# nayuki/DEFLATE-library-Java

Measured on AMD Instinct MI355X. Metric: input MiB/s (compress+decompress), higher is better.
Workload: dtype u8

## Files before the change

### deflate-library-java_amd/csrc/hip/inflate_wave.hpp

```cpp
#pragma once

namespace wv {
using namespace inf;

enum : uint32_t { K_LIT = 0, K_LEN = 1, K_EOB = 2, K_BAD = 3 };

struct Shared {
    Tabs t;
    uint8_t lens[320];
    uint16_t cl_tab[128];
    uint32_t exit_[64];
    uint8_t kind_[64];
    uint64_t h_pos, h_d0;
    uint32_t h_err, h_bfinal, h_btype, h_len, h_numlit, h_numdist;
};

struct PhArr {
    uint32_t cp[7][64];
    uint32_t end[7][64];
    uint32_t cnt[7][64];
    uint8_t kr[7][64];
};

__device__ __forceinline__ uint32_t lit_entry(uint32_t sym, uint32_t len) {
// ... 898 lines not shown
                tok_e<false>(lo[k], hi[k], en[k], p[k], t, ed, e, nb, tk);
                if (tk.kind > K_LEN) { l[k] = false; O[k].kr = tk.kind == K_EOB ? (T_EOB << 5) : ((T_ERR << 5) | tk.val); }
                else c[k] += tk.n;
            }
        }
    }
#pragma unroll
    for (int k = 0; k < N; k++) {
        Tok tk;
        if (l[k] && run_to(v, p[k], t, ed, e, nb, c[k], tk)) O[k].kr = tk.kind == K_EOB ? (T_EOB << 5) : ((T_ERR << 5) | tk.val);
        O[k].end = p[k]; O[k].cnt = c[k];
    }
}

__device__ __forceinline__ uint32_t esc_index(uint32_t lo, uint32_t hi, uint32_t esc4) {
    const uint32_t tl = (lo & esc4) ^ esc4, th = (hi & esc4) ^ esc4;
    const uint32_t zl = (tl - 0x01010101u) & ~tl & 0x80808080u, zh = (th - 0x01010101u) & ~th & 0x80808080u;
    return zl ? (uint32_t)__builtin_ctz(zl) >> 3 : zh ? 4u + ((uint32_t)__builtin_ctz(zh) >> 3) : 8u;
}
template <int N>
__device__ __forceinline__ void phase_multi_esc(const Lv& v, const Tabs& t, bool ed, uint32_t nb, uint32_t s0, uint32_t e,
                                                uint32_t esc4, PhOut (&O)[N]) {
    uint32_t p[N], c[N];
    bool l[N];
#pragma unroll
    for (int k = 0; k < N; k++) phase_first(v, t, ed, nb, s0 + k, e, p[k], c[k], O[k], l[k]);
    for (;;) {
        bool f[N], any = false;
#pragma unroll
        for (int k = 0; k < N; k++) { f[k] = l[k] && p[k] < e; any = any || f[k]; }
        if (!any) break;
        uint32_t lo[N], hi[N];
#pragma unroll
        for (int k = 0; k < N; k++) {
            const uint32_t pp = f[k] ? p[k] : p[0];
            const uint32_t* qk = v.p + ((pp >> 5) - v.rw) * 64;
            const uint32_t a = qk[0], wb = qk[64], cw = qk[128];
            lo[k] = __builtin_amdgcn_alignbit(wb, a, pp & 31);
            hi[k] = __builtin_amdgcn_alignbit(cw, wb, pp & 31);
        }
#pragma unroll
        for (int k = 0; k < N; k++) {
            if (!f[k]) continue;
            const uint32_t q = (e - p[k] + 7) >> 3, qi = (nb - min(nb, p[k])) >> 3;
            const uint32_t tt = min(min(esc_index(lo[k], hi[k], esc4), q), qi);
            if (tt) { p[k] += 8 * tt; c[k] += tt; continue; }
            Tok tk;
            tok_e<true>(lo[k], hi[k], t.lit[lo[k] & ((1u << LB) - 1u)], p[k], t, ed, e, nb, tk);
            if (tk.kind > K_LEN) { l[k] = false; O[k].kr = tk.kind == K_EOB ? (T_EOB << 5) : ((T_ERR << 5) | tk.val); }
            else c[k] += tk.n;
        }
    }
#pragma unroll
    for (int k = 0; k < N; k++) { O[k].end = p[k]; O[k].cnt = c[k]; }
}
__device__ __forceinline__ uint32_t flat8_mask(const Tabs& t, int lane) {
    uint64_t L[4];
#pragma unroll
    for (uint32_t i = 0; i < 4; i++) L[i] = __ballot((t.lit[(uint32_t)lane + 64 * i] & 0x800001FFu) == 0x80000088u);
    uint32_t m4 = 0;
#pragma unroll
    for (uint32_t kk = 0; kk < 3; kk++) {
        const uint32_t M = (1u << (8 - kk)) - 1u;
        bool same = true;
#pragma unroll
        for (uint32_t i = 0; i < 4; i++) same = same && __ballot((((uint32_t)lane + 64 * i) & M) != M) == L[i];
        if (same && !m4) m4 = M * 0x01010101u;
    }
    return m4;
}

__device__ __forceinline__ uint32_t sel8(const uint32_t (&v)[8], uint32_t i) {
    uint32_t r = v[0];
#pragma unroll
    for (uint32_t k = 1; k < 8; k++) r = i == k ? v[k] : r;
    return r;
}
__device__ __forceinline__ uint32_t phase_of(uint32_t d, uint32_t fbl, uint32_t fbh) {
    if (d < 8) return d;
    uint32_t r = 8;
#pragma unroll
    for (uint32_t f = 0; f < 8; f++) {
        const uint32_t fo = ((f < 4 ? fbl : fbh) >> (8 * (f & 3))) & 0xFFu;
        if (r == 8 && fo == d) r = f | 16u;
    }
    return r;
}
__device__ __forceinline__ uint32_t map_compose(uint32_t A, uint32_t B) {
    uint32_t r = 0;
#pragma unroll
    for (uint32_t f = 0; f < 8; f++) {
        const uint32_t bf = (B >> (4 * f)) & 15u;
        const uint32_t v = bf < 8 ? (A >> (4 * bf)) & 15u : 8u;
        r |= v << (4 * f);
    }
    return r;
}

__device__ __noinline__ void round_decode_phased(const In& in, const Tabs& t, bool ed, uint64_t rs, uint64_t E,
                                                 Shared& S, Stage& stg, int lane, Seg& out, uint32_t& first_term,
                                                 uint32_t& nfix, Geo& g, uint32_t esc4) {
    g = make_geo(in, rs, E);
    stage_round(in, g, stg, lane);
    const Lv v = make_lv(stg, g, lane);
    const uint32_t nb = g.nb;
    uint32_t s, e;
    lane_seg(g, lane, s, e);
    uint32_t endv[8], cntv[8], fbcv[8], krv[8];
    uint32_t fbl = 0, fbh = 0;
    constexpr uint32_t G = 2;
#pragma unroll 1
    for (uint32_t f = 0; f < 8; f += G) {
        PhOut P[G];
        if (esc4) phase_multi_esc<G>(v, t, ed, nb, s + f, e, esc4, P);
        else phase_multi<G>(v, t, ed, nb, s + f, e, P);
#pragma unroll
        for (uint32_t h = 0; h < G; h++) {
            const uint32_t g = f + h;
#pragma unroll
            for (uint32_t k = 0; k < 8; k++) {
                endv[k] = k == g ? P[h].end : endv[k];
                cntv[k] = k == g ? P[h].cnt : cntv[k];
                fbcv[k] = k == g ? P[h].fbc : fbcv[k];
                krv[k] = k == g ? P[h].kr : krv[k];
            }
            const uint32_t fo = (P[h].fb != NOCP && P[h].fb - s < 255u) ? P[h].fb - s : 255u;
            if (g < 4) fbl |= fo << (8 * g); else fbh |= fo << (8 * (g - 4));
        }
    }
    uint32_t Q = 0;
#pragma unroll
    for (uint32_t f = 0; f < 8; f++) {
        const uint32_t x = __shfl_up(endv[f], 1, 64);
        const uint32_t vv = phase_of(x - s, fbl, fbh) & 15u;
        if (lane > 0) Q |= vv << (4 * f);
    }
#pragma unroll
    for (int k = 1; k < 64; k <<= 1) {
        const uint32_t B = __shfl_up(Q, k, 64);
        if (lane >= k) Q = map_compose(Q, B);
    }
    const uint32_t myph = Q & 15u;
    const uint32_t xsel = myph < 8 ? sel8(endv, myph) : NOCP;
    uint32_t x = __shfl_up(xsel, 1, 64);
    if (lane == 0) x = s;
    SegR r;
    r.start = x; r.end = x; r.cnt = 0; r.kind = T_ERR; r.reason = R_INTERNAL;
    bool known = false;
    if (myph < 8) {
        const uint32_t pc = phase_of(x - s, fbl, fbh);
        const uint32_t f = pc & 15u;
        if (f == myph) {
            known = true;
            const uint32_t kr = sel8(krv, f);
            r.end = sel8(endv, f);
            r.cnt = sel8(cntv, f) - ((pc & 16u) ? sel8(fbcv, f) : 0u);
            r.kind = kr >> 5; r.reason = kr & 31u;
        }
    }
    const uint64_t km = __ballot(!known);
    const uint32_t u = km ? (uint32_t)__builtin_ctzll(km) : 64u;
    const uint64_t tm = __ballot(known && r.kind != T_EXIT);
    const uint32_t t0 = tm ? (uint32_t)__builtin_ctzll(tm) : 64u;
    first_term = min(t0, 64u);
    if (u < t0) {
        S.exit_[lane] = r.end;
        __syncthreads();
        first_term = 64;
        for (uint32_t j = u; j < 64 && first_term == 64; j++) {
            nfix++;
            if ((uint32_t)lane == j) {
                const uint32_t st = j ? (uint32_t)S.exit_[j - 1] : s;
                uint32_t en, cn, kr, fb, fbc;
                if (esc4) {
                    PhOut P1[1];
                    phase_multi_esc<1>(v, t, ed, nb, st, e, esc4, P1);
                    en = P1[0].end; cn = P1[0].cnt; kr = P1[0].kr;
                } else {
                    phase_run(v, t, ed, nb, st, e, en, cn, kr, fb, fbc);
                }
                r.start = st; r.end = en; r.cnt = cn; r.kind = kr >> 5; r.reason = kr & 31u;
                S.exit_[lane] = en;
                S.kind_[lane] = r.kind;
            }
            __syncthreads();
            if (S.kind_[j] != T_EXIT) first_term = j;
        }
    }
    out.start = g.base + r.start; out.end = g.base + r.end; out.cnt = r.cnt;
    out.kind = r.kind; out.reason = r.reason;
}

__device__ __forceinline__ uint64_t wave_sum_u64(uint64_t x) {
#pragma unroll
    for (int o = 32; o > 0; o >>= 1) x += __shfl_xor((unsigned long long)x, o, 64);
    return x;
}
__device__ __forceinline__ uint64_t wave_excl_u64(uint64_t v, int lane) {
    uint64_t x = v;
#pragma unroll
    for (int o = 1; o < 64; o <<= 1) {
        const uint64_t y = __shfl_up((unsigned long long)x, o, 64);
        if (lane >= o) x += y;
    }
    return x - v;
}

__device__ __forceinline__ bool is_cand(const uint64_t* cands, uint32_t ncand, uint64_t b, uint32_t* idx = nullptr) {
    uint32_t lo = 0, hi = ncand;
    while (lo < hi) { const uint32_t mid = (lo + hi) >> 1; if (cands[mid] < b) lo = mid + 1; else hi = mid; }
    if (idx) *idx = lo;
    return lo < ncand && cands[lo] == b;
}

__device__ __forceinline__ uint64_t next_cand(const uint64_t* cands, uint32_t ncand, uint64_t b, uint64_t limit) {
    uint32_t lo = 0, hi = ncand;
    while (lo < hi) { const uint32_t mid = (lo + hi) >> 1; if (cands[mid] <= b) lo = mid + 1; else hi = mid; }
    const uint64_t nx = lo < ncand ? cands[lo] : NONE;
    return min(nx, limit);
}

struct CandCur {
    const uint64_t* c;
    uint32_t n, i;
    uint64_t v;
    __device__ __forceinline__ void init(const uint64_t* cands, uint32_t ncand, uint64_t b) {
        c = cands; n = ncand;
        uint32_t lo = 0, hi = n;
        while (lo < hi) { const uint32_t mid = (lo + hi) >> 1; if (c[mid] < b) lo = mid + 1; else hi = mid; }
        i = lo;
        v = i < n ? c[i] : NONE;
    }
    __device__ __forceinline__ bool at(uint64_t b, uint32_t* idx) {
        while (v < b) { i++; v = i < n ? c[i] : NONE; }
        *idx = i;
        return v == b;
    }
    __device__ __forceinline__ uint64_t after(uint64_t b, uint64_t limit) {
        while (v <= b) { i++; v = i < n ? c[i] : NONE; }
        return min(v, limit);
    }
};

typedef __attribute__((address_space(1))) uint8_t gu8;
typedef __attribute__((address_space(1))) uint32_t gu32;
typedef __attribute__((address_space(1))) uint64_t gu64;

#ifdef NDFL_EMIT_NOSTORE
#define NDFL_OA(x) ((x) & 0xFFFull)
#else
#define NDFL_OA(x) (x)
#endif
typedef uint32_t u32x4v __attribute__((ext_vector_type(4)));
typedef __attribute__((address_space(1))) u32x4v gu128;
struct Wr {
    uint64_t acc;
    uint32_t an;
    uint64_t dst;
    uint32_t q0, q1, q2, hn;
};
__device__ __forceinline__ void wr_init(Wr& w, uint64_t dst) {
    w.acc = 0; w.an = 0; w.dst = dst;
    w.q0 = 0; w.q1 = 0; w.q2 = 0; w.hn = 0;
}
__device__ __forceinline__ void wr_drain(Wr& w, gu8* out) {
    if (w.hn) {
        gu8* d = out + NDFL_OA(w.dst - 4 * w.hn);
        if (w.hn >= 2) *(gu64*)d = (uint64_t)w.q0 | ((uint64_t)w.q1 << 32);
        if (w.hn == 1) *(gu32*)d = w.q0;
        if (w.hn == 3) *(gu32*)(d + 8) = w.q2;
        w.hn = 0;
    }
}
__device__ __forceinline__ void wr_lit(Wr& w, gu8* out, uint32_t val, uint32_t n) {
    w.acc |= (uint64_t)val << (8 * w.an);
    w.an += n;
    if (w.an >= 4) {
        const uint32_t word = (uint32_t)w.acc;
        if (w.hn == 3) {
            *(gu128*)(out + NDFL_OA(w.dst - 12)) = u32x4v{w.q0, w.q1, w.q2, word};
            w.hn = 0;
        } else {
            w.q0 = w.hn == 0 ? word : w.q0;
            w.q1 = w.hn == 1 ? word : w.q1;
            w.q2 = w.hn == 2 ? word : w.q2;
            w.hn++;
        }
        w.acc >>= 32;
        w.an -= 4;
        w.dst += 4;
    }
}
__device__ __forceinline__ void wr_flush_word(Wr& w, gu8* out) {
    wr_drain(w, out);
    if (w.an) {
        *(gu32*)(out + NDFL_OA(w.dst)) = (uint32_t)w.acc;
        w.dst += w.an;
        w.acc = 0;
        w.an = 0;
    }
}
__device__ __forceinline__ void wr_flush_exact(Wr& w, gu8* out) {
    wr_drain(w, out);
    for (uint32_t k = 0; k < w.an; k++) out[NDFL_OA(w.dst + k)] = (uint8_t)(w.acc >> (8 * k));
    w.dst += w.an;
    w.acc = 0;
    w.an = 0;
}
__device__ __forceinline__ uint64_t ld8(const gu8* p) { return *(const gu64*)p; }
__device__ __forceinline__ uint32_t ld4(const gu8* p) { return *(const gu32*)p; }
__device__ __forceinline__ void wr_copy(gu8* out, uint64_t dst, uint32_t len, uint32_t dist, uint32_t& lastb) {
    gu8* d = out + NDFL_OA(dst);
    const gu8* sp = out + NDFL_OA(dst - dist);
    if (dist == 1) {
        const uint32_t v4 = lastb * 0x01010101u;
        if (len >= 16) {
            const u32x4v x = {v4, v4, v4, v4};
            uint32_t k = 0;
            for (; k + 16 <= len; k += 16) *(gu128*)(d + k) = x;
            if (k < len) *(gu128*)(d + len - 16) = x;
            return;
        }
        if (len >= 4) {
            uint32_t k = 0;
            for (; k + 4 <= len; k += 4) *(gu32*)(d + k) = v4;
            if (k < len) *(gu32*)(d + len - 4) = v4;
        } else {
            for (uint32_t k = 0; k < len; k++) d[k] = (uint8_t)lastb;
        }
        return;
    }
    if (dist >= 16 && len >= 16) {
        uint32_t k = 0;
        u32x4v x = {0, 0, 0, 0};
        for (; k + 16 <= len; k += 16) { x = *(const gu128*)(sp + k); *(gu128*)(d + k) = x; }
        if (k < len) { x = *(const gu128*)(sp + len - 16); *(gu128*)(d + len - 16) = x; }
        lastb = x.w >> 24;
        return;
    }
    if (dist >= 8 && len >= 8) {
        uint32_t k = 0;
        uint64_t x = 0;
        for (; k + 8 <= len; k += 8) { x = ld8(sp + k); *(gu64*)(d + k) = x; }
        if (k < len) { x = ld8(sp + len - 8); *(gu64*)(d + len - 8) = x; }
        lastb = (uint32_t)(x >> 56);
        return;
    }
    if (dist >= 4 && len >= 4) {
        uint32_t k = 0, x = 0;
        for (; k + 4 <= len; k += 4) { x = ld4(sp + k); *(gu32*)(d + k) = x; }
        if (k < len) { x = ld4(sp + len - 4); *(gu32*)(d + len - 4) = x; }
        lastb = x >> 24;
        return;
    }
    uint32_t b = lastb;
    for (uint32_t k = 0; k < len; k++) { b = sp[k]; d[k] = (uint8_t)b; }
    lastb = b;
}

}

extern "C" __global__ void __launch_bounds__(64)
ndfl_inflate_hdr_kernel(const uint32_t* w, uint64_t nwords, uint64_t nbits, const uint64_t* cands, uint32_t ncand,
                        wv::HdrRec* rec, uint32_t* flat_list, uint32_t* nflat, uint32_t* flat_flag) {
    using namespace wv;
    __shared__ __attribute__((aligned(16))) uint32_t lens[64][80];
    __shared__ uint16_t clt[64][128];
    __shared__ uint32_t win[8 * 64];
    const uint32_t lane = threadIdx.x;
    const uint32_t k = blockIdx.x * 64 + lane;
    if (k >= ncand) return;
    const In in{w, nwords, nbits};
    for (uint32_t q = 0; q < 80; q++) lens[lane][q] = 0;
    const uint64_t p = cands[k];
    Hdr h;
    parse_hdr_core<RdWin>(in, p, (uint8_t*)lens[lane], clt[lane], h, win + lane);
    HdrRec* r = rec + k;
    for (uint32_t q = 0; q < 80; q += 4)
        *(uint4*)&r->lens[q] = make_uint4(lens[lane][q], lens[lane][q + 1], lens[lane][q + 2], lens[lane][q + 3]);
    r->h = h;
    r->at = p;
    uint32_t c8 = 0;
    bool bad = false;
    for (uint32_t q = 0; q < 72; q++) {
        const uint32_t v = lens[lane][q];
#pragma unroll
        for (uint32_t b = 0; b < 4; b++) {
            const uint32_t l = (v >> (8 * b)) & 0xFFu;
            c8 += l == 8 ? 1u : 0u;
            bad = bad || (l - 1u < 7u) || (l == 8 && q >= 64);
        }
    }
    const uint32_t esc = 256u - min(c8, 256u);
    const uint32_t kk = esc == 1 ? 1u : esc == 2 ? 2u : esc == 4 ? 3u : 0u;
    r->flat = (flat_list && h.err == 0 && h.btype == 2 && !bad) ? kk : 0u;
    r->pad = 0;
    if (flat_flag) flat_flag[k] = r->flat;
    if (flat_list) {
        const uint64_t m = __ballot(r->flat != 0);
        uint32_t b = 0;
        if (lane == 0 && m) b = atomicAdd(nflat, (uint32_t)__popcll(m));
        b = __shfl(b, 0, 64);
        if (r->flat) flat_list[b + (uint32_t)__popcll(m & ((1ull << lane) - 1ull))] = k;
    }
}

#ifndef NDFL_COUNT_WPE
#define NDFL_COUNT_WPE 3
#endif
namespace wv {
#ifndef NDFL_FLAT_OTHER_MAX
#define NDFL_FLAT_OTHER_MAX 64
#endif
#ifndef NDFL_FLAT_K
#define NDFL_FLAT_K 4
#endif
#ifndef NDFL_FLAT_PRIO
#define NDFL_FLAT_PRIO 1
#endif
#ifdef NDFL_FLAT_PROF
__device__ unsigned long long g_flat_prof[4];
#endif
constexpr uint32_t FLAT_ESC_WORD = 64;
static_assert(FLAT_ESC_WORD + 64 * 64 / 4 <= SW * 64, "flat escape tables in the stage");

__device__ __forceinline__ uint32_t flat_esc_entry(const TabsG& t, uint32_t kk, uint32_t x) {
    const uint32_t pl = 8 - kk;
    const uint32_t w = ((1u << pl) - 1u) | (x << pl);
    uint32_t e = t.lit[w & ((1u << LB) - 1u)];
    uint32_t len, kind;
    if (e >> 31) {
        len = e & 15; kind = 0;
    } else {
        if (!(e & 31)) e = long_lit(e, w, t);
        len = e & 31;
        const uint32_t k = (e >> 9) & 3;
        kind = k == K_LIT ? 0u : k == K_EOB ? 1u : 2u;
    }
    return (kind < 2 && len > pl && len <= pl + 6) ? (len | (kind << 4)) : 0u;
}

__device__ __forceinline__ uint32_t count_flat_group(const In& in, const uint32_t* flist, uint32_t n,
                                                     const uint64_t* cands, uint32_t ncand, uint64_t limit,
                                                     uint64_t stop_all, ChainRes* res, const SegPool& pool,
                                                     const HdrRec* hrec, Shared& S, uint32_t* stw, int lane,
                                                     uint32_t* redo, uint32_t& tb_next, uint32_t& tb_end,
                                                     uint32_t* whys) {
    lu8* escs = (lu8*)((lu32*)stw + FLAT_ESC_WORD);
    uint32_t my_c = 0, my_brec = NOREC, my_kk = 0;
    uint64_t my_d0 = 0;
    bool my_ok = false, my_final = false, my_ed = false;
    for (uint32_t k = 0; k < n; k++) {
        const uint32_t c = flist[k];
        const HdrRec* hr = hrec + c;
        uint32_t* lw = (uint32_t*)S.lens;
        lw[lane] = hr->lens[lane];
        if (lane < 16) lw[64 + lane] = hr->lens[64 + lane];
        if (lane == 0) hdr_to_shared(hr->h, S);
        const uint32_t kk = hr->flat - 1u;
        __syncthreads();
        bool ed;
        const int te = build_tables(S, lane, ed, stw);
        uint32_t brec = NOREC;
        if (!te) {
            if (c < pool.nslot && pool.nbt) {
                brec = claim_table_record(pool, tb_next, tb_end, lane);
                if (brec != NOREC)
                    write_table_record(pool, brec, S.t, cands[c], S.h_d0, S.h_bfinal, S.h_btype, ed,
                                       ((1u << (8 - kk)) - 1u) * 0x01010101u,
                                       (uint32_t)lane, 64);
            }
            const TabsG tg{S.t.lit, S.t.dst, S.t.lx, S.t.dx};
            escs[k * 64 + lane] = (uint8_t)flat_esc_entry(tg, kk, (uint32_t)lane);
        }
        if ((uint32_t)lane == k) {
            my_c = c; my_ok = !te; my_d0 = S.h_d0; my_final = S.h_bfinal != 0; my_ed = ed; my_brec = brec; my_kk = kk;
        }
        __syncthreads();
    }
    const bool active = (uint32_t)lane < n && my_ok;
    uint32_t ci = my_c;
    uint64_t cv = active ? cands[ci] : NONE;
    auto after = [&](uint64_t b) {
        while (cv <= b) { ci++; cv = ci < ncand ? cands[ci] : NONE; }
        return min(cv, limit);
    };
    uint32_t nr = 0;
    if (active) {
        const uint64_t e0 = after(my_d0);
        nr = (uint32_t)min<uint64_t>((e0 > my_d0 ? (e0 - my_d0 + MAX_SPAN - 1) / MAX_SPAN : 1) + 1, 1024);
    }
    uint64_t cv1 = NONE, cv2 = NONE, cv3 = NONE;
    if (active) {
        cv1 = ci + 1 < ncand ? cands[ci + 1] : NONE;
        cv2 = ci + 2 < ncand ? cands[ci + 2] : NONE;
        cv3 = ci + 3 < ncand ? cands[ci + 3] : NONE;
    }
    const uint32_t rpre = (uint32_t)wave_excl_u64(nr, lane), rtot = (uint32_t)wave_sum_u64(nr);
    uint32_t rb = 0;
    if (lane == 0 && rtot) rb = atomicAdd(pool.ctr, rtot);
    rb = __builtin_amdgcn_readfirstlane(rb);
    bool ok = false;
    uint64_t total = 0, endpos = 0;
    uint32_t status = ST_BOUNDARY, next_idx = 0xFFFFFFFFu, why = active ? 4u : 5u;
    if (active) {
        const uint32_t pl = 8 - my_kk, M4 = ((1u << pl) - 1u) * 0x01010101u;
        bool recording = my_c < pool.nslot;
        uint32_t rnext = rb + rpre, rlast = rnext + nr;
        uint32_t brec = my_brec, others = 0;
        const uint64_t o64 = (my_d0 >> 8) << 8;
        const uint64_t og4 = o64 >> 7;
        const uint32_t nbo = (uint32_t)min<uint64_t>(in.nbits - min(in.nbits, o64), 0xFFFFFF00ull);
        uint32_t pos = (uint32_t)(my_d0 - o64);
        lu32* ring = (lu32*)&S.t + lane;
        uint32_t fw = (pos >> 5) & ~7u;
#pragma unroll
        for (uint32_t i = 0; i < 24; i += 4) {
            const u32x4 v = in.ld4(og4 + ((fw + i) >> 2));
            ring[i * 64] = v.x; ring[(i + 1) * 64] = v.y; ring[(i + 2) * 64] = v.z; ring[(i + 3) * 64] = v.w;
        }
        fw += 24;
        uint32_t frow = 0;
        u32x4 ra = in.ld4(og4 + (fw >> 2)), rb = in.ld4(og4 + (fw >> 2) + 1);
        uint32_t base = 0, r0 = 0, re = 0, per = 0, pw = 0, nbr = 0, idx = NOREC, j = 0, p = 0, jst = 0, bytes = 0, sn = 0;
        uint64_t* ps = nullptr;
        uint32_t* pc = nullptr;
        SegMeta* mp = nullptr;
        uint32_t* link = pool.head + my_c;
        uint32_t st = 0;
        if (NDFL_FLAT_PRIO) __builtin_amdgcn_s_setprio(3);
        auto end_round = [&](bool eob) {
            if (ps) {
                const uint64_t ex = o64 + base + p;
                ps[j] = o64 + base + jst;
                pc[j] = bytes;
                for (uint32_t jj = j + 1; jj < 64; jj++) { ps[jj] = ex; pc[jj] = 0; }
                uint32_t kf = eob ? (uint32_t)T_EOB : (uint32_t)T_EXIT;
                asm volatile("" : "+v"(kf));
                write_round_meta(mp, eob ? j : 64u, kf, 0u, NOREC, ex, ex, pw, brec, o64 + base + r0);
                *link = idx;
                link = &mp->next;
                brec = NOREC;
            }
            total += bytes;
            pos = base + p;
        };
#ifdef NDFL_FLAT_PROF
        unsigned long long fp_ph = 0, fp_t0 = clock64(), fp_n = 0;
#endif
        while (st < 2) {
            {
#ifdef NDFL_FLAT_PROF
                const unsigned long long fp_a = clock64();
#endif
                const uint32_t cw = (st == 1 ? base + p : pos) >> 5;
                if (cw + 16 >= fw) {
                    ring[frow * 64] = ra.x; ring[(frow + 1) * 64] = ra.y; ring[(frow + 2) * 64] = ra.z;
                    ring[(frow + 3) * 64] = ra.w; ring[(frow + 4) * 64] = rb.x; ring[(frow + 5) * 64] = rb.y;
                    ring[(frow + 6) * 64] = rb.z; ring[(frow + 7) * 64] = rb.w;
                    fw += 8;
                    frow = frow == 16 ? 0u : frow + 8;
                    ra = in.ld4(og4 + (fw >> 2)); rb = in.ld4(og4 + (fw >> 2) + 1);
                }
#ifdef NDFL_FLAT_PROF
                asm volatile("s_waitcnt lgkmcnt(0)" ::: "memory");
                fp_ph += clock64() - fp_a;
                fp_n++;
#endif
            }
            for (uint32_t k = 0; k < NDFL_FLAT_K && st < 2; k++) {
                if (st == 0) {
                    const uint64_t rsa = o64 + pos;
                    if (cv <= rsa) { cv = cv1; cv1 = cv2; cv2 = cv3; cv3 = NONE; ci++; }
                    if (cv <= rsa) {
                        while (cv <= rsa) { ci++; cv = ci < ncand ? cands[ci] : NONE; }
                        cv1 = ci + 1 < ncand ? cands[ci + 1] : NONE;
                        cv2 = ci + 2 < ncand ? cands[ci + 2] : NONE;
                        cv3 = ci + 3 < ncand ? cands[ci + 3] : NONE;
                    }
                    uint64_t E = min(min(cv, limit), rsa + MAX_SPAN);
                    if (E <= rsa) E = rsa + 1;
                    base = pos & ~31u;
                    r0 = pos - base; re = (uint32_t)(E - o64) - base;
                    pw = seg_pw(re - r0); per = pw * 32;
                    nbr = nbo - min(nbo, base);
                    idx = NOREC;
                    if (recording) {
                        if (rnext >= rlast) {
                            rnext = atomicAdd(pool.ctr, 8u);
                            rlast = rnext + 8;
                        }
                        if (rnext < pool.nrec) idx = rnext++;
                        else recording = false;
                    }
                    ps = idx != NOREC ? pool.start + (uint64_t)idx * 64 : nullptr;
                    pc = idx != NOREC ? pool.cnt + (uint64_t)idx * 64 : nullptr;
                    mp = idx != NOREC ? pool.meta + idx : nullptr;
                    j = 0; p = r0; jst = r0; bytes = 0;
                    sn = seg_end(r0, per, re, 0);
                    st = 1;
                }
                if (st != 1) continue;
                const uint32_t ap = base + p, cw = ap >> 5;
                const bool tk_ok = p < sn && cw + 2 < fw;
                uint32_t rr0 = frow + 24 - min(fw - cw, 24u);
                rr0 = rr0 >= 24 ? rr0 - 24 : rr0;
// ... 214 lines not shown
                        rb_next = b; rb_end = b + NDFL_REC_BATCH;
                    }
                    idx = rb_next++;
                }
                if (idx < pool.nrec) {
                    pool.start[(uint64_t)idx * 64 + lane] = r.start;
                    pool.cnt[(uint64_t)idx * 64 + lane] = (uint32_t)r.cnt;
                    const int src = ft < 64 ? (int)ft : 63;
                    const uint64_t fe = __shfl((unsigned long long)r.end, src, 64);
                    const uint32_t fk = __shfl(r.kind, src, 64), fr = __shfl(r.reason, src, 64);
                    if (lane == 0) {
                        SegMeta m;
                        m.ft = ft; m.kind_ft = fk; m.reason_ft = fr; m.next = NOREC;
                        m.end_ft = fe; m.exit63 = fe; m.pw = g.pw; m.brec = brec; m.rs = g.base + g.r0;
                        pool.meta[idx] = m;
                        if (prev_rec == NOREC) pool.head[slot_base + c] = idx;
                        else pool.meta[prev_rec].next = idx;
                    }
                    prev_rec = idx;
                    brec = NOREC;
                } else {
                    recording = false;
                }
            }
            nround++;
            if (pc) { const uint64_t x = wall_clock64(); pc->rec += x - tb; tb = x; }
            total += wave_sum_u64((uint32_t)lane <= ft ? r.cnt : 0ull);
            if (ft < 64) {
                const uint64_t fe = __shfl((unsigned long long)r.end, (int)ft, 64);
                const uint32_t fk = __shfl(r.kind, (int)ft, 64), fr = __shfl(r.reason, (int)ft, 64);
                block_done = true;
                if (fk == T_ERR) { status = ST_ERROR; reason = fr; endpos = fe; chain_done = true; }
                else {
                    cur = fe;
                    if (bfinal) { status = ST_FINAL; endpos = cur; chain_done = true; }
                }
            } else {
                rs = __shfl((unsigned long long)r.end, 63, 64);
            }
        }
        if (chain_done) break;
    }
    if (lane == 0) {
        ChainRes o;
        o.end_bit = endpos; o.out_count = total; o.status = status; o.reason = reason;
        o.next = next_idx;
        o.pad = stats ? (min((uint32_t)((wall_clock64() - t_chain) / 1000), 0xFFFFu) << 16) | min(nblk + 1, 0xFFFFu) : 0u;
        o.bnd_bit = 0; o.bnd_cnt = 0;
        res[c] = o;
        if (stats) {
            atomicAdd(&stats[SW_NSLOW], nslow); atomicAdd(&stats[SW_NFIX], nfix); atomicAdd(&stats[SW_NROUND], nround);
            unsigned long long* st64 = (unsigned long long*)(stats + SW_CLOCK64);
            atomicAdd(&st64[0], pcl.hdr); atomicAdd(&st64[1], pcl.spec); atomicAdd(&st64[2], pcl.verify);
            atomicAdd(&st64[3], pcl.phases); atomicAdd(&st64[4], pcl.serial); atomicAdd(&st64[5], pcl.rec);
            atomicAdd(&st64[6], pcl.build); atomicAdd(&st64[7], pcl.phmap);
            atomicMax(&st64[12], (unsigned long long)(wall_clock64() - t_chain));
        }
    }
    }
    if (stats && lane == 0) {
        unsigned long long* st64 = (unsigned long long*)(stats + SW_CLOCK64);
        const uint64_t t_end = wall_clock64();
        atomicAdd(&st64[8], t_end - t_begin);
        atomicMax(&st64[9], t_end);
        atomicMax(&st64[10], ~t_begin);
        atomicAdd(&st64[11], 1ull);
    }
}

#ifndef NDFL_EMIT_WAVES_PER_SIMD
#define NDFL_EMIT_WAVES_PER_SIMD 3
#endif
extern "C" __global__ void __launch_bounds__(64) __attribute__((amdgpu_waves_per_eu(NDFL_EMIT_WAVES_PER_SIMD)))
ndfl_inflate_emit_wave_kernel(const uint32_t* w, uint64_t nwords, uint64_t nbits, const EmitChain* chains,
                              uint32_t nlist, uint32_t* ticket, uint8_t* out, ChainRes* res, const uint64_t* cands,
                              uint32_t ncand, uint32_t* ref, uint32_t* pend, SegPool pool, wv::PhArr* ph_all,
                              uint32_t* stats, const uint64_t* info, const uint32_t* eorder,
                              const uint32_t* dnlist) {
    using namespace wv;
    __shared__ __attribute__((aligned(16))) Shared S;
    __shared__ Stage stg;
    __shared__ uint32_t s_ticket;
    const int lane = threadIdx.x;
    gu8* gout = (gu8*)out;
    PhArr* S_ph = ph_all + blockIdx.x;
    const uint64_t t_begin = stats ? wall_clock64() : 0;
    if (info) {
        if (info[LI_FLAGS]) return;
        nlist = (uint32_t)info[LI_NCH];
    }
    if (dnlist) {
        nlist = *dnlist;
        if (nlist == 0) return;
    }
    for (;;) {
    __syncthreads();
    if (lane == 0) s_ticket = atomicAdd(ticket, 1u);
    __syncthreads();
    if (s_ticket >= nlist) break;
    const uint32_t ci = eorder ? eorder[s_ticket] : s_ticket;
    const In in{w, nwords, nbits};
    const EmitChain ch = chains[ci];
    const uint64_t t_chain = stats ? wall_clock64() : 0;
    uint64_t cur = ch.start_bit, base = ch.out_off;
    uint32_t status = ST_BOUNDARY, reason = 0;
    uint64_t endpos = ch.start_bit;
    uint32_t nslow = 0, nfix = 0;
    uint32_t rec = ch.slot < pool.nslot ? pool.head[ch.slot] : NOREC;
    SegMeta pm = {};
    uint64_t pst = 0;
    uint32_t pcn = 0;
    rec_fetch(pool, rec, lane, pm, pst, pcn);
    uint64_t bnd_bit = cur, bnd_out = base;
    for (int blk = 0;; blk++) {
        if (blk > 0 && cur == ch.end_bit) { status = ST_BOUNDARY; endpos = cur; break; }
        bnd_bit = cur; bnd_out = base;
        const TabRec* btr = block_tables(pool, rec, pm, cur);
        if (btr) {
            __syncthreads();
            const uint4* src = (const uint4*)&btr->t;
            uint4* dst = (uint4*)&S.t;
            for (uint32_t q = (uint32_t)lane; q < sizeof(Tabs) / 16; q += 64) dst[q] = src[q];
            if (lane == 0) {
                S.h_err = 0; S.h_d0 = btr->data_bit; S.h_bfinal = btr->bfinal; S.h_btype = btr->btype; S.h_len = btr->ed;
            }
            __syncthreads();
        } else {
            for (uint32_t s = (uint32_t)lane; s < 320; s += 64) S.lens[s] = 0;
            __syncthreads();
            if (lane == 0) parse_hdr(in, cur, S);
            __syncthreads();
        }
        if (S.h_err) { status = ST_ERROR; reason = S.h_err; endpos = S.h_pos; break; }
        const uint64_t d0 = S.h_d0;
        const bool bfinal = S.h_bfinal != 0;
        if (S.h_btype == 0) {
            const uint64_t avail = (nbits - d0) / 8, ln = S.h_len;
            const uint64_t take = min(avail, ln);
            const uint64_t ib = d0 >> 3;
            for (uint64_t i = (uint64_t)lane; i < take; i += 64) {
                const uint64_t b = ib + i;
                out[base + i] = (uint8_t)(in.ld(b >> 2) >> (8 * (uint32_t)(b & 3)));
            }
            base += take;
            if (take < ln) { status = ST_ERROR; reason = R_UEOS; endpos = d0 + 8 * avail; break; }
            cur = d0 + 8 * ln;
            if (bfinal) { status = ST_FINAL; endpos = cur; break; }
            continue;
        }
        bool ed;
        if (btr) {
            ed = S.h_len != 0;
        } else {
            const int te = build_tables(S, lane, ed, stg.w);
            if (te) { status = ST_ERROR; reason = (uint32_t)te; endpos = d0; break; }
        }
        uint64_t rs = d0;
        bool block_done = false, chain_done = false;
        while (!block_done) {
            Seg r;
            uint32_t ft;
            Geo g;
            if (rec != NOREC) {
                const SegMeta m = pm;
                ft = m.ft;
                r.start = pst;
                r.cnt = pcn;
                rec = m.next;
                rec_fetch(pool, rec, lane, pm, pst, pcn);
                round_lane_end(m, r.start, lane, r.end, r.kind, r.reason);
                g = make_geo(in, m.rs, m.rs + 1, m.pw);
                stage_round(in, g, stg, lane);
            } else {
                uint64_t E = min(next_cand(cands, ncand, rs, ch.end_bit), rs + MAX_SPAN);
                if (E <= rs) E = rs + 1;
                round_decode(in, S.t, ed, rs, E, S, stg, lane, r, ft, nslow, nfix, S_ph, g);
            }
            const bool live = (uint32_t)lane <= ft;
            const uint64_t mycnt = live ? r.cnt : 0ull;
            const uint64_t pre = wave_excl_u64(mycnt, lane);
            const uint64_t rsum = wave_sum_u64(mycnt);
            const Lv v = make_lv(stg, g, lane);
            const uint32_t nb = g.nb;
            uint32_t pos = (uint32_t)(r.start - g.base);
            uint32_t end = (uint32_t)(r.end - g.base);
            uint32_t kind = r.kind, rsn = r.reason;
            const uint64_t dst0 = base + pre;
            uint32_t n = 0;
            Wr wr;
            wr_init(wr, dst0);
            uint64_t dfr = ~0ull;
            uint64_t lastsrc = 0;
            bool lsp = false;
            uint32_t lastb = 0;
            bool lastok = false;
            bool active = live;
            Bb bb;
            const uint32_t lim = min(end, nb - min(nb, 48u));
            bool fast = active && pos < lim;
            if (fast) bb_init(bb, v, pos);
            while (active && pos < end) {
                Tok tk;
                if (fast) {
                    tok_bb<true>(bb, v, S.t, ed, tk, end);
                    pos = bb.pos;
                    fast = pos < lim;
                } else {
                    tok<true>(v, pos, S.t, ed, end, nb, tk);
                }
                if (tk.kind == K_LIT) {
                    wr_lit(wr, gout, tk.val, tk.n);
                    n += tk.n;
                    lsp = true;
                    lastb = tk.val >> (tk.n == 2 ? 8 : 0);
                    lastok = true;
                    continue;
                }
                if (tk.kind != K_LEN) break;
                const uint64_t dst = dst0 + n;
                if ((uint64_t)tk.dist > dst) {
                    kind = T_ERR; rsn = R_COPY_BEFORE; end = pos; break;
                }
                const uint32_t len = tk.n, dist = tk.dist;
                const uint64_t src = dst - dist;
                const uint64_t src_end = src + min(len, dist);
                bool defer = src < dst0;
                if (!defer && src_end > dfr) {
                    for (uint64_t q = src >> 5; q <= (src_end - 1) >> 5 && !defer; q++) {
                        const uint64_t lo = max(src, q << 5), hi = min(src_end, (q + 1) << 5);
                        const uint32_t m = (uint32_t)(((1ull << (hi - lo)) - 1) << (lo & 31));
                        defer = (__hip_atomic_load(&pend[q], __ATOMIC_RELAXED, __HIP_MEMORY_SCOPE_AGENT) & m) != 0;
                    }
                }
                wr_flush_word(wr, gout);
                if (!defer && dist == 1 && !lastok) lastb = gout[dst - 1];
                if (!defer) {
                    wr_copy(gout, dst, len, dist, lastb);
                    lastok = true;
                    lsp = true;
                } else {
                    const uint64_t anchor = dist == 1 ? (n > 0 ? (lsp ? dst - 1 : lastsrc) : src) : 0;
                    for (uint32_t k = 0; k < len; k++) {
                        const uint64_t back = dst + k - anchor;
                        ref[dst + k] = dist == 1 ? (back < (1ull << 32) ? (uint32_t)back : 1u) : dist;
                    }
                    for (uint64_t q = dst >> 5; q <= (dst + len - 1) >> 5; q++) {
                        const uint64_t lo = max(dst, q << 5), hi = min(dst + len, (q + 1) << 5);
                        const uint32_t m = (uint32_t)(((1ull << (hi - lo)) - 1) << (lo & 31));
                        atomicOr(&pend[q], m);
                    }
                    lastsrc = anchor;
                    lsp = dist != 1;
                    dfr = min(dfr, dst);
                    lastok = false;
                }
                n += len;
                wr.dst = dst0 + n;
            }
            wr_flush_exact(wr, gout);
            if (live && kind != T_ERR && (n != mycnt || pos != end)) { kind = T_ERR; rsn = R_INTERNAL; }
            const uint64_t em = __ballot(live && kind == T_ERR);
            if (em) {
                const int fl = (int)__builtin_ctzll(em);
                status = ST_ERROR;
                reason = __shfl(rsn, fl, 64);
                endpos = g.base + __shfl(end, fl, 64);
                base = __shfl((unsigned long long)(dst0 + n), fl, 64);
                chain_done = true;
                break;
            }
            base += rsum;
            if (ft < 64) {
                block_done = true;
                cur = __shfl((unsigned long long)r.end, (int)ft, 64);
                if (bfinal) { status = ST_FINAL; endpos = cur; chain_done = true; }
            } else {
                rs = __shfl((unsigned long long)r.end, 63, 64);
            }
        }
        if (chain_done) break;
    }
    if (lane == 0) {
        ChainRes o;
        o.end_bit = endpos; o.out_count = base - ch.out_off; o.status = status; o.reason = reason;
        o.next = 0xFFFFFFFFu; o.pad = 0;
        o.bnd_bit = bnd_bit; o.bnd_cnt = bnd_out - ch.out_off;
        res[ci] = o;
        if (stats) atomicMax((unsigned long long*)(stats + SW_CLOCK64) + 20, (unsigned long long)(wall_clock64() - t_chain));
    }
    }
    if (stats && lane == 0) {
        unsigned long long* st64 = (unsigned long long*)(stats + SW_CLOCK64);
        const uint64_t t_end = wall_clock64();
        atomicAdd(&st64[16], t_end - t_begin);
        atomicMax(&st64[17], t_end);
        atomicMax(&st64[18], ~t_begin);
        atomicAdd(&st64[19], 1ull);
    }
}

#ifndef NDFL_EMITF_WAVES_PER_SIMD
#define NDFL_EMITF_WAVES_PER_SIMD 4
#endif
extern "C" __global__ void __launch_bounds__(64) __attribute__((amdgpu_waves_per_eu(NDFL_EMITF_WAVES_PER_SIMD)))
ndfl_inflate_emit_fast_kernel(const uint32_t* w, uint64_t nwords, uint64_t nbits, const EmitChain* chains,
                              uint32_t* ticket, uint8_t* out, ChainRes* res, uint32_t* ref, uint32_t* pend,
                              SegPool pool, const uint64_t* info, const uint32_t* eorder, uint32_t* slow,
                              uint32_t* nslow) {
    using namespace wv;
    __shared__ __attribute__((aligned(16))) uint32_t Tp[(1u << LB) + (1u << DB)];
    TabsG T;
    T.lit = Tp;
    T.dst = Tp + (1u << LB);
    __shared__ Stage stg;
    const int lane = threadIdx.x;
    gu8* gout = (gu8*)out;
    if (info[LI_FLAGS]) return;
    const uint32_t nlist = (uint32_t)info[LI_NCH];
    const In in{w, nwords, nbits};
    for (;;) {
    uint32_t tk0 = 0;
    if (lane == 0) tk0 = atomicAdd(ticket, 1u);
    const uint32_t t = __builtin_amdgcn_readfirstlane(tk0);
    if (t >= nlist) break;
    const uint32_t ci = eorder[t];
    const EmitChain ch = chains[ci];
    uint64_t cur = ch.start_bit, base = ch.out_off;
    uint32_t status = ST_BOUNDARY, reason = 0;
    uint64_t endpos = ch.start_bit;
    bool abort = false;
    uint32_t rec = ch.slot < pool.nslot ? pool.head[ch.slot] : NOREC;
    SegMeta pm = {};
    uint64_t pst = 0;
    uint32_t pcn = 0;
    rec_fetch(pool, rec, lane, pm, pst, pcn);
    uint64_t bnd_bit = cur, bnd_out = base;
    for (int blk = 0;; blk++) {
        if (blk > 0 && cur == ch.end_bit) { status = ST_BOUNDARY; endpos = cur; break; }
        bnd_bit = cur; bnd_out = base;
        if (cur + 3 > nbits) { abort = true; break; }
        const uint32_t hb = (uint32_t)(in.win64(cur)) & 7u;
        if ((hb >> 1) == 0) {
            const uint64_t hp = (cur + 3 + 7) & ~7ull;
            if (hp + 32 > nbits) { abort = true; break; }
            const uint32_t lw = (uint32_t)in.win64(hp);
            if ((lw >> 16) != (~lw & 0xFFFFu)) { abort = true; break; }
            const uint64_t ln = lw & 0xFFFFu, d0 = hp + 32;
            if (d0 + 8 * ln > nbits) { abort = true; break; }
            const uint64_t ib = d0 >> 3;
            for (uint64_t i = (uint64_t)lane; i < ln; i += 64) {
                const uint64_t b = ib + i;
                out[base + i] = (uint8_t)(in.ld(b >> 2) >> (8 * (uint32_t)(b & 3)));
            }
            base += ln;
            cur = d0 + 8 * ln;
            if (hb & 1) { status = ST_FINAL; endpos = cur; break; }
            continue;
        }
        const TabRec* btr = block_tables(pool, rec, pm, cur);
        if (!btr) { abort = true; break; }
        __syncthreads();
        {
            static_assert(offsetof(Tabs, lit) == 0 && offsetof(Tabs, dst) == sizeof(Tp) - sizeof(btr->t.dst), "primary tables first");
            const uint4* src = (const uint4*)&btr->t;
            uint4* dst = (uint4*)Tp;
            for (uint32_t q = (uint32_t)lane; q < sizeof(Tp) / 16; q += 64) dst[q] = src[q];
            const TabsG tv = tabs_view(btr);
            T.lx = tv.lx;
            T.dx = tv.dx;
        }
        const bool bfinal = btr->bfinal != 0, ed = btr->ed != 0;
        const uint32_t tph = btr->phase;
        const bool ph8 = tph != TP_NONE;
        const uint32_t esc4 = tph > TP_LIT8 ? tph : 0u;
        __syncthreads();
        bool block_done = false, chain_done = false;
        while (!block_done) {
            if (rec == NOREC) { abort = true; chain_done = true; break; }
            const SegMeta m = pm;
            const uint32_t ft = m.ft;
            const uint64_t rstart = pst;
            const uint32_t rcnt = pcn;
            rec = m.next;
            rec_fetch(pool, rec, lane, pm, pst, pcn);
            uint64_t rend;
            uint32_t kind, rsn;
            round_lane_end(m, rstart, lane, rend, kind, rsn);
            const Geo g = make_geo(in, m.rs, m.rs + 1, m.pw);
            const bool live = (uint32_t)lane <= ft;
            const uint64_t mycnt = live ? rcnt : 0ull;
            const uint64_t pre = wave_excl_u64(mycnt, lane);
            const uint64_t rsum = wave_sum_u64(mycnt);
            stage_round(in, g, stg, lane);
            const Lv v = make_lv(stg, g, lane);
            const uint32_t nb = g.nb;
            uint32_t pos = (uint32_t)(rstart - g.base);
            uint32_t end = (uint32_t)(rend - g.base);
            const uint64_t dst0 = base + pre;
            uint32_t n = 0;
            Wr wr;
            wr_init(wr, dst0);
            uint64_t dfr = ~0ull, lastsrc = 0;
            bool lsp = false;
            uint32_t lastb = 0;
            bool lastok = false;
            Bb bb;
            const uint32_t lim = min(end, nb - min(nb, 48u));
            bool fast = live && pos < lim;
            if (fast) bb_init(bb, v, pos);
            auto token_loop = [&](auto ph) {
                using PH = decltype(ph);
                while (live && pos < end) {
                    Tok tk;
                    if (PH::value && fast && esc4) {
                        const uint32_t lo = (uint32_t)bb.buf, hi = (uint32_t)(bb.buf >> 32);
                        const uint32_t t = min(min(esc_index(lo, hi, esc4), bb.nb >> 3), (end - pos + 7) >> 3);
                        if (t) {
                            uint32_t b[8];
#pragma unroll
                            for (uint32_t i = 0; i < 8; i++)
                                b[i] = (T.lit[(i < 4 ? lo >> (8 * i) : hi >> (8 * (i - 4))) & 0xFFu] >> 9) & 0xFFu;
                            const uint32_t v0 = b[0] | (b[1] << 8) | (b[2] << 16) | (b[3] << 24);
                            const uint32_t v1 = b[4] | (b[5] << 8) | (b[6] << 16) | (b[7] << 24);
                            const uint32_t n0 = min(t, 4u);
                            wr_lit(wr, gout, n0 == 4 ? v0 : v0 & ((1u << (8 * n0)) - 1u), n0);
                            if (t > 4) wr_lit(wr, gout, t == 8 ? v1 : v1 & ((1u << (8 * (t - 4))) - 1u), t - 4);
                            n += t;
                            lsp = true;
                            lastb = t > 4 ? (v1 >> (8 * (t - 5))) & 0xFFu : (v0 >> (8 * (t - 1))) & 0xFFu;
                            lastok = true;
                            bb.buf = t < 8 ? bb.buf >> (8 * t) : 0ull;
                            bb.nb -= 8 * t;
                            bb.pos += 8 * t;
                            bb_refill(bb, v);
                            pos = bb.pos;
                            fast = pos < lim;
                            continue;
                        }
                    }
                    if (PH::value && fast && !esc4 && bb.nb >= 34 && pos + 24 < end) {
                        const uint32_t lo = (uint32_t)bb.buf, hi = (uint32_t)(bb.buf >> 32);
                        const uint32_t e0 = T.lit[lo & ((1u << LB) - 1u)], e1 = T.lit[(lo >> 8) & ((1u << LB) - 1u)];
                        const uint32_t e2 = T.lit[(lo >> 16) & ((1u << LB) - 1u)];
                        const uint32_t e3 = T.lit[__builtin_amdgcn_alignbit(hi, lo, 24) & ((1u << LB) - 1u)];
                        if (((e0 & 0x800001FFu) == 0x80000088u) && ((e1 & 0x800001FFu) == 0x80000088u) &&
                            ((e2 & 0x800001FFu) == 0x80000088u) && ((e3 & 0x800001FFu) == 0x80000088u)) {
                            const uint32_t b3 = (e3 >> 9) & 0xFFu;
                            wr_lit(wr, gout, ((e0 >> 9) & 0xFFu) | (((e1 >> 9) & 0xFFu) << 8) | (((e2 >> 9) & 0xFFu) << 16) | (b3 << 24), 4);
                            n += 4;
                            lsp = true;
                            lastb = b3;
                            lastok = true;
                            bb_skip(bb, 32);
                            bb_refill(bb, v);
                            pos = bb.pos;
                            fast = pos < lim;
                            continue;
                        }
                    }
                    if (fast) {
                        tok_bb<true>(bb, v, T, ed, tk, end);
                        pos = bb.pos;
                        fast = pos < lim;
                    } else {
                        tok<true>(v, pos, T, ed, end, nb, tk);
                    }
                    if (tk.kind == K_LIT) {
                        wr_lit(wr, gout, tk.val, tk.n);
                        n += tk.n;
                        lsp = true;
                        lastb = tk.val >> (tk.n == 2 ? 8 : 0);
                        lastok = true;
                        continue;
                    }
                    if (tk.kind != K_LEN) break;
                    const uint64_t dst = dst0 + n;
                    if ((uint64_t)tk.dist > dst) { kind = T_ERR; rsn = R_COPY_BEFORE; end = pos; break; }
                    const uint32_t len = tk.n, dist = tk.dist;
                    const uint64_t src = dst - dist;
                    const uint64_t src_end = src + min(len, dist);
                    bool defer = src < dst0;
                    if (!defer && src_end > dfr) {
                        for (uint64_t q = src >> 5; q <= (src_end - 1) >> 5 && !defer; q++) {
                            const uint64_t lo = max(src, q << 5), hi = min(src_end, (q + 1) << 5);
                            const uint32_t mk = (uint32_t)(((1ull << (hi - lo)) - 1) << (lo & 31));
                            defer = (__hip_atomic_load(&pend[q], __ATOMIC_RELAXED, __HIP_MEMORY_SCOPE_AGENT) & mk) != 0;
                        }
                    }
                    wr_flush_word(wr, gout);
                    if (!defer && dist == 1 && !lastok) lastb = gout[dst - 1];
                    if (!defer) {
                        wr_copy(gout, dst, len, dist, lastb);
                        lastok = true;
                        lsp = true;
                    } else {
                        const uint64_t anchor = dist == 1 ? (n > 0 ? (lsp ? dst - 1 : lastsrc) : src) : 0;
                        for (uint32_t k = 0; k < len; k++) {
                            const uint64_t back = dst + k - anchor;
                            ref[dst + k] = dist == 1 ? (back < (1ull << 32) ? (uint32_t)back : 1u) : dist;
                        }
                        for (uint64_t q = dst >> 5; q <= (dst + len - 1) >> 5; q++) {
                            const uint64_t lo = max(dst, q << 5), hi = min(dst + len, (q + 1) << 5);
                            const uint32_t mk = (uint32_t)(((1ull << (hi - lo)) - 1) << (lo & 31));
                            atomicOr(&pend[q], mk);
                        }
                        lastsrc = anchor;
                        lsp = dist != 1;
                        dfr = min(dfr, dst);
                        lastok = false;
                    }
                    n += len;
                    wr.dst = dst0 + n;
                }
            };
            if (ph8) token_loop(std::true_type{}); else token_loop(std::false_type{});
            wr_flush_exact(wr, gout);
            if (live && kind != T_ERR && (n != rcnt || pos != end)) { kind = T_ERR; rsn = R_INTERNAL; }
            const uint64_t em = __ballot(live && kind == T_ERR);
            if (em) {
                const int fl = (int)__builtin_ctzll(em);
                status = ST_ERROR;
                reason = __shfl(rsn, fl, 64);
                endpos = g.base + __shfl(end, fl, 64);
                base = __shfl((unsigned long long)(dst0 + n), fl, 64);
                chain_done = true;
                break;
            }
            base += rsum;
            if (ft < 64) {
                block_done = true;
                cur = __shfl((unsigned long long)rend, (int)ft, 64);
                if (bfinal) { status = ST_FINAL; endpos = cur; chain_done = true; }
            }
        }
        if (chain_done) break;
    }
    if (lane == 0) {
        if (abort) {
            slow[atomicAdd(nslow, 1u)] = ci;
        } else {
            ChainRes o;
            o.end_bit = endpos; o.out_count = base - ch.out_off; o.status = status; o.reason = reason;
            o.next = 0xFFFFFFFFu; o.pad = 0;
            o.bnd_bit = bnd_bit; o.bnd_cnt = bnd_out - ch.out_off;
            res[ci] = o;
        }
    }
    }
}

#ifndef NDFL_RESOLVE_HOPS
#define NDFL_RESOLVE_HOPS 4
#endif
extern "C" __global__ void __launch_bounds__(256)
ndfl_inflate_resolve_kernel(const uint32_t* list, const uint32_t* nlist, const uint32_t* pend, uint32_t* ref,
                            uint8_t* out, uint32_t* newbits) {
    const uint32_t n = *nlist;
    const uint32_t b = threadIdx.x & 31;
    for (uint32_t k = (blockIdx.x * 256 + threadIdx.x) >> 5; k < n; k += gridDim.x * 8) {
        const uint64_t wd = list[k];
        const uint32_t bits = pend[wd];
        bool still = false;
        if ((bits >> b) & 1) {
            const uint64_t i = wd * 32 + b;
            uint64_t d = ref[i];
            uint64_t p = i - d;
            bool pending = (pend[p >> 5] >> (p & 31)) & 1;
#pragma unroll 1
            for (int h = 1; h < NDFL_RESOLVE_HOPS && pending; h++) {
                const uint64_t nd = d + ref[p];
                if (nd >= (1ull << 32)) break;
                d = nd;
                p = i - d;
                pending = (pend[p >> 5] >> (p & 31)) & 1;
            }
            if (pending) {
                const uint64_t nd = d + ref[p];
                ref[i] = (uint32_t)(nd < (1ull << 32) ? nd : d);
                still = true;
            } else {
                out[i] = out[p];
            }
        }
        const uint64_t m = __ballot(still);
        if (b == 0) newbits[k] = (uint32_t)(m >> (threadIdx.x & 32));
    }
}

__device__ __forceinline__ void block_append(bool flag, uint32_t v, uint32_t* list, uint32_t* n) {
    __shared__ uint32_t wc[4], wbase;
    const int lane = threadIdx.x & 63, wid = threadIdx.x >> 6;
    const uint64_t m = __ballot(flag);
    if (lane == 0) wc[wid] = (uint32_t)__popcll(m);
    __syncthreads();
    if (threadIdx.x == 0) {
        const uint32_t t = wc[0] + wc[1] + wc[2] + wc[3];
        wbase = t ? atomicAdd(n, t) : 0u;
    }
    __syncthreads();
    uint32_t off = wbase;
    for (int k = 0; k < wid; k++) off += wc[k];
    if (flag) list[off + __popcll(m & ((1ull << lane) - 1))] = v;
    __syncthreads();
}

extern "C" __global__ void __launch_bounds__(256)
ndfl_inflate_resolve_apply_kernel(const uint32_t* list, const uint32_t* nlist, uint32_t* pend, const uint32_t* newbits,
                                  uint32_t* list_out, uint32_t* nlist_out, uint32_t* nbytes_out) {
    const uint32_t n = *nlist;
    for (uint32_t k0 = blockIdx.x * 256; k0 < n; k0 += gridDim.x * 256) {
        const uint32_t k = k0 + threadIdx.x;
        const bool live = k < n;
        uint32_t nb = 0, wd = 0;
        if (live) { wd = list[k]; nb = newbits[k]; pend[wd] = nb; }
        if (nbytes_out) {
            const uint32_t c = wave_sum((uint32_t)__popc(nb));
            if ((threadIdx.x & 63) == 0 && c) atomicAdd(nbytes_out, c);
        }
        block_append(live && nb != 0, wd, list_out, nlist_out);
    }
}

extern "C" __global__ void __launch_bounds__(256)
ndfl_inflate_pending_list_kernel(const uint32_t* pend, uint64_t w0, uint64_t w1, uint32_t* list, uint32_t* nlist) {
    __shared__ uint32_t sh[4], sbase;
    const uint64_t base = w0 + ((uint64_t)blockIdx.x * 256 + threadIdx.x) * 16;
    uint32_t v[16];
    if (base + 16 <= w1 && (base & 3) == 0) {
        const u32x4* q = (const u32x4*)(pend + base);
#pragma unroll
        for (int k = 0; k < 4; k++) { const u32x4 x = q[k]; v[4 * k] = x.x; v[4 * k + 1] = x.y; v[4 * k + 2] = x.z; v[4 * k + 3] = x.w; }
    } else {
#pragma unroll
        for (int k = 0; k < 16; k++) v[k] = base + k < w1 ? pend[base + k] : 0u;
    }
    uint32_t cnt = 0;
#pragma unroll
    for (int k = 0; k < 16; k++) cnt += v[k] != 0;
    uint32_t tot;
    const uint32_t off = block_excl_scan<uint32_t, 4>(cnt, sh, tot);
    if (threadIdx.x == 0) sbase = tot ? atomicAdd(nlist, tot) : 0u;
    __syncthreads();
    uint32_t o = sbase + off;
#pragma unroll
    for (int k = 0; k < 16; k++)
        if (v[k]) list[o++] = (uint32_t)(base + k);
}
```

Measured before the change: 217,600.

## Batch literal runs in inner loop with branchless shift-register writer

```diff
diff --git a/deflate-library-java_amd/csrc/hip/inflate_wave.hpp b/deflate-library-java_amd/csrc/hip/inflate_wave.hpp
--- a/deflate-library-java_amd/csrc/hip/inflate_wave.hpp
+++ b/deflate-library-java_amd/csrc/hip/inflate_wave.hpp
@@ -1224,6 +1224,45 @@
 }
 __device__ __forceinline__ void wr_flush_exact(Wr& w, gu8* out) {
     wr_drain(w, out);
+    for (uint32_t k = 0; k < w.an; k++) out[NDFL_OA(w.dst + k)] = (uint8_t)(w.acc >> (8 * k));
+    w.dst += w.an;
+    w.acc = 0;
+    w.an = 0;
+}
+__device__ __forceinline__ void wrs_lit(Wr& w, gu8* out, uint32_t val, uint32_t n) {
+    w.acc |= (uint64_t)val << (8 * w.an);
+    w.an += n;
+    const bool full = w.an >= 4;
+    const uint32_t word = (uint32_t)w.acc;
+    if (full && w.hn == 3) *(gu128*)(out + NDFL_OA(w.dst - 12)) = u32x4v{w.q0, w.q1, w.q2, word};
+    w.q0 = full ? w.q1 : w.q0;
+    w.q1 = full ? w.q2 : w.q1;
+    w.q2 = full ? word : w.q2;
+    w.hn = (w.hn + (full ? 1u : 0u)) & 3u;
+    w.acc = full ? w.acc >> 32 : w.acc;
+    w.an &= 3u;
+    w.dst += full ? 4u : 0u;
+}
+__device__ __forceinline__ void wrs_drain(Wr& w, gu8* out) {
+    if (w.hn) {
+        gu8* d = out + NDFL_OA(w.dst - 4 * w.hn);
+        if (w.hn == 1) *(gu32*)d = w.q2;
+        if (w.hn == 2) *(gu64*)d = (uint64_t)w.q1 | ((uint64_t)w.q2 << 32);
+        if (w.hn == 3) { *(gu64*)d = (uint64_t)w.q0 | ((uint64_t)w.q1 << 32); *(gu32*)(d + 8) = w.q2; }
+        w.hn = 0;
+    }
+}
+__device__ __forceinline__ void wrs_flush_word(Wr& w, gu8* out) {
+    wrs_drain(w, out);
+    if (w.an) {
+        *(gu32*)(out + NDFL_OA(w.dst)) = (uint32_t)w.acc;
+        w.dst += w.an;
+        w.acc = 0;
+        w.an = 0;
+    }
+}
+__device__ __forceinline__ void wrs_flush_exact(Wr& w, gu8* out) {
+    wrs_drain(w, out);
     for (uint32_t k = 0; k < w.an; k++) out[NDFL_OA(w.dst + k)] = (uint8_t)(w.acc >> (8 * k));
     w.dst += w.an;
     w.acc = 0;
@@ -2044,6 +2083,9 @@
 #ifndef NDFL_EMITF_WAVES_PER_SIMD
 #define NDFL_EMITF_WAVES_PER_SIMD 4
 #endif
+#ifndef NDFL_EMITF_LITRUN_K
+#define NDFL_EMITF_LITRUN_K 8
+#endif
 extern "C" __global__ void __launch_bounds__(64) __attribute__((amdgpu_waves_per_eu(NDFL_EMITF_WAVES_PER_SIMD)))
 ndfl_inflate_emit_fast_kernel(const uint32_t* w, uint64_t nwords, uint64_t nbits, const EmitChain* chains,
                               uint32_t* ticket, uint8_t* out, ChainRes* res, uint32_t* ref, uint32_t* pend,
@@ -2153,53 +2195,66 @@
             auto token_loop = [&](auto ph) {
                 using PH = decltype(ph);
                 while (live && pos < end) {
-                    Tok tk;
-                    if (PH::value && fast && esc4) {
-                        const uint32_t lo = (uint32_t)bb.buf, hi = (uint32_t)(bb.buf >> 32);
-                        const uint32_t t = min(min(esc_index(lo, hi, esc4), bb.nb >> 3), (end - pos + 7) >> 3);
-                        if (t) {
-                            uint32_t b[8];
-#pragma unroll
-                            for (uint32_t i = 0; i < 8; i++)
-                                b[i] = (T.lit[(i < 4 ? lo >> (8 * i) : hi >> (8 * (i - 4))) & 0xFFu] >> 9) & 0xFFu;
-                            const uint32_t v0 = b[0] | (b[1] << 8) | (b[2] << 16) | (b[3] << 24);
-                            const uint32_t v1 = b[4] | (b[5] << 8) | (b[6] << 16) | (b[7] << 24);
-                            const uint32_t n0 = min(t, 4u);
-                            wr_lit(wr, gout, n0 == 4 ? v0 : v0 & ((1u << (8 * n0)) - 1u), n0);
-                            if (t > 4) wr_lit(wr, gout, t == 8 ? v1 : v1 & ((1u << (8 * (t - 4))) - 1u), t - 4);
-                            n += t;
+                    if (fast) {
+#pragma unroll 1
+                        for (uint32_t k = 0; k < NDFL_EMITF_LITRUN_K; k++) {
+                            if (PH::value && bb.pos >= lim) break;
+                            if (PH::value && esc4) {
+                                const uint32_t lo = (uint32_t)bb.buf, hi = (uint32_t)(bb.buf >> 32);
+                                const uint32_t t = min(min(esc_index(lo, hi, esc4), bb.nb >> 3), (end - bb.pos + 7) >> 3);
+                                if (t) {
+                                    uint32_t b[8];
+#pragma unroll
+                                    for (uint32_t i = 0; i < 8; i++)
+                                        b[i] = (T.lit[(i < 4 ? lo >> (8 * i) : hi >> (8 * (i - 4))) & 0xFFu] >> 9) & 0xFFu;
+                                    const uint32_t v0 = b[0] | (b[1] << 8) | (b[2] << 16) | (b[3] << 24);
+                                    const uint32_t v1 = b[4] | (b[5] << 8) | (b[6] << 16) | (b[7] << 24);
+                                    const uint32_t n0 = min(t, 4u);
+                                    wrs_lit(wr, gout, n0 == 4 ? v0 : v0 & ((1u << (8 * n0)) - 1u), n0);
+                                    if (t > 4) wrs_lit(wr, gout, t == 8 ? v1 : v1 & ((1u << (8 * (t - 4))) - 1u), t - 4);
+                                    lastb = ((t > 4 ? (v1 >> (8 * (t - 5))) & 0xFFu : (v0 >> (8 * (t - 1))) & 0xFFu) << 9);
+                                    bb.buf = t < 8 ? bb.buf >> (8 * t) : 0ull;
+                                    bb.nb -= 8 * t;
+                                    bb.pos += 8 * t;
+                                    bb_refill(bb, v);
+                                    continue;
+                                }
+                            }
+                            if (PH::value && !esc4 && bb.nb >= 34 && bb.pos + 24 < end) {
+                                const uint32_t lo = (uint32_t)bb.buf, hi = (uint32_t)(bb.buf >> 32);
+                                const uint32_t e0 = T.lit[lo & ((1u << LB) - 1u)], e1 = T.lit[(lo >> 8) & ((1u << LB) - 1u)];
+                                const uint32_t e2 = T.lit[(lo >> 16) & ((1u << LB) - 1u)];
+                                const uint32_t e3 = T.lit[__builtin_amdgcn_alignbit(hi, lo, 24) & ((1u << LB) - 1u)];
+                                if (((e0 & 0x800001FFu) == 0x80000088u) && ((e1 & 0x800001FFu) == 0x80000088u) &&
+                                    ((e2 & 0x800001FFu) == 0x80000088u) && ((e3 & 0x800001FFu) == 0x80000088u)) {
+                                    wrs_lit(wr, gout, ((e0 >> 9) & 0xFFu) | (((e1 >> 9) & 0xFFu) << 8) | (((e2 >> 9) & 0xFFu) << 16) | (((e3 >> 9) & 0xFFu) << 24), 4);
+                                    lastb = e3;
+                                    bb_skip(bb, 32);
+                                    bb_refill(bb, v);
+                                    continue;
+                                }
+                            }
+                            const uint32_t e = T.lit[(uint32_t)bb.buf & ((1u << LB) - 1u)];
+                            if (!((e >> 31) && bb.pos + 2u * LB < lim)) break;
+                            wrs_lit(wr, gout, (e >> 9) & 0xFFFFu, 1u + ((e >> 8) & 1u));
+                            lastb = e;
+                            bb_skip(bb, e & 15);
+                            bb_refill(bb, v);
+                        }
+                        pos = bb.pos;
+                        const uint32_t nn = (uint32_t)(wr.dst - dst0) + wr.an;
+                        if (nn != n) {
                             lsp = true;
-                            lastb = t > 4 ? (v1 >> (8 * (t - 5))) & 0xFFu : (v0 >> (8 * (t - 1))) & 0xFFu;
+                            lastb = (lastb >> ((lastb >> 8) & 1u ? 17 : 9)) & 0xFFu;
                             lastok = true;
-                            bb.buf = t < 8 ? bb.buf >> (8 * t) : 0ull;
-                            bb.nb -= 8 * t;
-                            bb.pos += 8 * t;
-                            bb_refill(bb, v);
-                            pos = bb.pos;
+                            n = nn;
+                        }
+                        if (PH::value) {
                             fast = pos < lim;
-                            continue;
+                            if (pos >= end) break;
                         }
                     }
-                    if (PH::value && fast && !esc4 && bb.nb >= 34 && pos + 24 < end) {
-                        const uint32_t lo = (uint32_t)bb.buf, hi = (uint32_t)(bb.buf >> 32);
-                        const uint32_t e0 = T.lit[lo & ((1u << LB) - 1u)], e1 = T.lit[(lo >> 8) & ((1u << LB) - 1u)];
-                        const uint32_t e2 = T.lit[(lo >> 16) & ((1u << LB) - 1u)];
-                        const uint32_t e3 = T.lit[__builtin_amdgcn_alignbit(hi, lo, 24) & ((1u << LB) - 1u)];
-                        if (((e0 & 0x800001FFu) == 0x80000088u) && ((e1 & 0x800001FFu) == 0x80000088u) &&
-                            ((e2 & 0x800001FFu) == 0x80000088u) && ((e3 & 0x800001FFu) == 0x80000088u)) {
-                            const uint32_t b3 = (e3 >> 9) & 0xFFu;
-                            wr_lit(wr, gout, ((e0 >> 9) & 0xFFu) | (((e1 >> 9) & 0xFFu) << 8) | (((e2 >> 9) & 0xFFu) << 16) | (b3 << 24), 4);
-                            n += 4;
-                            lsp = true;
-                            lastb = b3;
-                            lastok = true;
-                            bb_skip(bb, 32);
-                            bb_refill(bb, v);
-                            pos = bb.pos;
-                            fast = pos < lim;
-                            continue;
-                        }
-                    }
+                    Tok tk;
                     if (fast) {
                         tok_bb<true>(bb, v, T, ed, tk, end);
                         pos = bb.pos;
@@ -2208,7 +2263,7 @@
                         tok<true>(v, pos, T, ed, end, nb, tk);
                     }
                     if (tk.kind == K_LIT) {
-                        wr_lit(wr, gout, tk.val, tk.n);
+                        wrs_lit(wr, gout, tk.val, tk.n);
                         n += tk.n;
                         lsp = true;
                         lastb = tk.val >> (tk.n == 2 ? 8 : 0);
@@ -2229,7 +2284,7 @@
                             defer = (__hip_atomic_load(&pend[q], __ATOMIC_RELAXED, __HIP_MEMORY_SCOPE_AGENT) & mk) != 0;
                         }
                     }
-                    wr_flush_word(wr, gout);
+                    wrs_flush_word(wr, gout);
                     if (!defer && dist == 1 && !lastok) lastb = gout[dst - 1];
                     if (!defer) {
                         wr_copy(gout, dst, len, dist, lastb);
@@ -2256,7 +2311,7 @@
                 }
             };
             if (ph8) token_loop(std::true_type{}); else token_loop(std::false_type{});
-            wr_flush_exact(wr, gout);
+            wrs_flush_exact(wr, gout);
             if (live && kind != T_ERR && (n != rcnt || pos != end)) { kind = T_ERR; rsn = R_INTERNAL; }
             const uint64_t em = __ballot(live && kind == T_ERR);
             if (em) {
```

Result: faster. 227,700 (median of 6 runs) (+4.6%).
